# zengyan-97/X2-VLM

Hardware: AMD Instinct MI355X
Metric: image-text pairs/sec (fwd+bwd) X2VLM-base 224px bs=64/GPU (higher is better)
Workload: dtype bf16

## Files before the change

x2-vlm_amd/csrc/rowwise.hip:

```cpp
#include "x2_common.h"

__device__ __forceinline__ long remap_row(int r, int period) { return period > 0 ? (long)r + r / period + 1 : r; }

#define LN_MAXV 8
#define LN_DISPATCH(D, CALL) do { const int nv_ = ((D) + 255) / 256; \
  if (nv_ <= 1) { CALL(1); } else if (nv_ == 2) { CALL(2); } else if (nv_ == 3) { CALL(3); } else if (nv_ == 4) { CALL(4); } \
  else if (nv_ <= 6) { CALL(6); } else { CALL(8); } } while (0)
template <int NV>
__global__ __launch_bounds__(256) void layernorm_fwd_kernel(const float* __restrict__ x, const float* __restrict__ w,
                                                            const float* __restrict__ bsh, bf16_t* yb, float* yf,
                                                            float* mean, float* rstd, int rows, int D, float eps, int period,
                                                            DropSpec drop_in_, const uint32_t* __restrict__ epoch) {
  const int row = blockIdx.x * 4 + (threadIdx.x >> 6), lane = threadIdx.x & 63;
  if (row >= rows) return;
  const DropSpec drop = drop_at_epoch(drop_in_, epoch);
  const long gr = remap_row(row, period);
  const float* xr = x + gr * D;
  float4 v[NV];
  float s = 0.f;
  const int nv = D >> 2;
#pragma unroll
  for (int i = 0; i < NV; ++i) {
    const int c = lane + i * 64;
    if (c < nv) { v[i] = *reinterpret_cast<const float4*>(xr + c * 4); s += v[i].x + v[i].y + v[i].z + v[i].w; }
  }
  const float mu = wave_sum(s) / D;
  float q = 0.f;
#pragma unroll
  for (int i = 0; i < NV; ++i) {
    const int c = lane + i * 64;
    if (c < nv) { const float a = v[i].x - mu, b = v[i].y - mu, cc = v[i].z - mu, d = v[i].w - mu; q += a * a + b * b + cc * cc + d * d; }
  }
  const float rs = rsqrtf(wave_sum(q) / D + eps);
  if (lane == 0) { mean[row] = mu; rstd[row] = rs; }
#pragma unroll
  for (int i = 0; i < NV; ++i) {
    const int c = lane + i * 64;
    if (c < nv) {
      const float4 ww = *reinterpret_cast<const float4*>(w + c * 4), bb = *reinterpret_cast<const float4*>(bsh + c * 4);
      float4 o{(v[i].x - mu) * rs * ww.x + bb.x, (v[i].y - mu) * rs * ww.y + bb.y, (v[i].z - mu) * rs * ww.z + bb.z, (v[i].w - mu) * rs * ww.w + bb.w};
      if (drop.thr16) {
        float dm[4];
        drop_mul4(drop, (uint32_t)gr * (uint32_t)D + (uint32_t)(c * 4), dm);
        o.x *= dm[0]; o.y *= dm[1]; o.z *= dm[2]; o.w *= dm[3];
      }
      if (yf) *reinterpret_cast<float4*>(yf + gr * D + c * 4) = o;
      if (yb) *reinterpret_cast<u32x2*>(yb + gr * D + c * 4) = u32x2{pack_bf16(o.x, o.y), pack_bf16(o.z, o.w)};
    }
  }
}

template <int NV, int RPW>
__global__ __launch_bounds__(256) void layernorm_fwd_rows_kernel(const float* __restrict__ x, const float* __restrict__ w,
                                                                 const float* __restrict__ bsh, bf16_t* yb, float* yf,
                                                                 float* mean, float* rstd, int rows, int D, float eps, int period,
                                                                 DropSpec drop_in_, const uint32_t* __restrict__ epoch) {
  const int row0 = (blockIdx.x * 4 + (threadIdx.x >> 6)) * RPW, lane = threadIdx.x & 63;
  if (row0 >= rows) return;
  const DropSpec drop = drop_at_epoch(drop_in_, epoch);
  const int nv = D >> 2;
  float4 v[RPW][NV];
  long gr[RPW];
#pragma unroll
  for (int r = 0; r < RPW; ++r) {
    const int row = min(row0 + r, rows - 1);
    gr[r] = remap_row(row, period);
#pragma unroll
    for (int i = 0; i < NV; ++i) {
      const int c = lane + i * 64;
      v[r][i] = c < nv ? *reinterpret_cast<const float4*>(x + gr[r] * D + c * 4) : float4{0.f, 0.f, 0.f, 0.f};
    }
  }
  float4 ww[NV], bb[NV];
#pragma unroll
  for (int i = 0; i < NV; ++i) {
    const int c = lane + i * 64;
    ww[i] = c < nv ? *reinterpret_cast<const float4*>(w + c * 4) : float4{0.f, 0.f, 0.f, 0.f};
    bb[i] = c < nv ? *reinterpret_cast<const float4*>(bsh + c * 4) : float4{0.f, 0.f, 0.f, 0.f};
  }
#pragma unroll
  for (int r = 0; r < RPW; ++r) {
    float s = 0.f;
#pragma unroll
    for (int i = 0; i < NV; ++i) if (lane + i * 64 < nv) s += v[r][i].x + v[r][i].y + v[r][i].z + v[r][i].w;
    const float mu = wave_sum(s) / D;
    float q = 0.f;
#pragma unroll
    for (int i = 0; i < NV; ++i)
      if (lane + i * 64 < nv) { const float a = v[r][i].x - mu, b = v[r][i].y - mu, cc = v[r][i].z - mu, d = v[r][i].w - mu; q += a * a + b * b + cc * cc + d * d; }
    const float rs = rsqrtf(wave_sum(q) / D + eps);
    if (row0 + r >= rows) continue;
    if (lane == 0) { mean[row0 + r] = mu; rstd[row0 + r] = rs; }
#pragma unroll
    for (int i = 0; i < NV; ++i) {
      const int c = lane + i * 64;
      if (c < nv) {
        float4 o{(v[r][i].x - mu) * rs * ww[i].x + bb[i].x, (v[r][i].y - mu) * rs * ww[i].y + bb[i].y,
                 (v[r][i].z - mu) * rs * ww[i].z + bb[i].z, (v[r][i].w - mu) * rs * ww[i].w + bb[i].w};
        if (drop.thr16) {
          float dm[4];
          drop_mul4(drop, (uint32_t)gr[r] * (uint32_t)D + (uint32_t)(c * 4), dm);
          o.x *= dm[0]; o.y *= dm[1]; o.z *= dm[2]; o.w *= dm[3];
        }
        if (yf) *reinterpret_cast<float4*>(yf + gr[r] * D + c * 4) = o;
        if (yb) *reinterpret_cast<u32x2*>(yb + gr[r] * D + c * 4) = u32x2{pack_bf16(o.x, o.y), pack_bf16(o.z, o.w)};
      }
    }
  }
}

extern "C" int x2_tune_get(int key);
extern "C" int x2_layernorm_fwd(const float* x, const float* w, const float* b, void* y_bf16, float* y_f32, float* mean,
                                float* rstd, int rows, int D, float eps, int period, unsigned drop_thr16, unsigned drop_seed,
                                float drop_scale, const unsigned* drop_epoch, void* stream) {
  X2_REQUIRE(rows > 0 && D > 0 && D % 4 == 0 && D <= 256 * LN_MAXV, "x2_layernorm_fwd: rows=%d D=%d (D%%4==0, D<=2048)", rows, D);
#define X2_LNF(NV) hipLaunchKernelGGL(layernorm_fwd_kernel<NV>, dim3((rows + 3) / 4), dim3(256), 0, (hipStream_t)stream, x, w, b, \
                     (bf16_t*)y_bf16, y_f32, mean, rstd, rows, D, eps, period, DropSpec{drop_thr16, drop_seed, drop_scale}, drop_epoch)
#define X2_LNF_R(NV, RPW) hipLaunchKernelGGL((layernorm_fwd_rows_kernel<NV, RPW>), dim3((rows + 4 * RPW - 1) / (4 * RPW)), dim3(256), 0, (hipStream_t)stream, \
                     x, w, b, (bf16_t*)y_bf16, y_f32, mean, rstd, rows, D, eps, period, DropSpec{drop_thr16, drop_seed, drop_scale}, drop_epoch)
  const int knob = x2_tune_get(13), nvv = (D + 255) / 256;
  int rpw = knob == 1 || knob == 2 || knob == 4 ? knob : (rows >= 8 * 4 * 256 ? 2 : 1);
  if (nvv > 4) rpw = 1;
  if (rpw == 4 && nvv <= 3) { if (nvv <= 1) X2_LNF_R(1, 4); else if (nvv == 2) X2_LNF_R(2, 4); else X2_LNF_R(3, 4); }
  else if (rpw >= 2) { if (nvv <= 1) X2_LNF_R(1, 2); else if (nvv == 2) X2_LNF_R(2, 2); else if (nvv == 3) X2_LNF_R(3, 2); else X2_LNF_R(4, 2); }
  else LN_DISPATCH(D, X2_LNF);
  return x2_check_launch("x2_layernorm_fwd");
}

__global__ __launch_bounds__(256) void reduce_partials_kernel(const float* __restrict__ part, int nblk, int nk, int width,
                                                              float* o0, float* o1, float* o2, float* o3 = nullptr) {
  const int c = blockIdx.x * 64 + (threadIdx.x & 63), k = blockIdx.y, sl = threadIdx.x >> 6;
  __shared__ float red[3][64];
  float s = 0.f;
  if (c < width) {
#pragma unroll 4
    for (int b = sl; b < nblk; b += 4) s += part[((long)b * nk + k) * width + c];
  }
  if (sl > 0) red[sl - 1][threadIdx.x & 63] = s;
  __syncthreads();
  if (sl == 0 && c < width) {
    float* o = k == 0 ? o0 : (k == 1 ? o1 : (k == 2 ? o2 : o3));
    if (o) o[c] += s + red[0][threadIdx.x] + red[1][threadIdx.x] + red[2][threadIdx.x];
  }
}
static void launch_reduce(const float* part, int nblk, int nk, int width, float* o0, float* o1, float* o2, hipStream_t st, float* o3 = nullptr) {
  hipLaunchKernelGGL(reduce_partials_kernel, dim3((width + 63) / 64, nk), dim3(256), 0, st, part, nblk, nk, width, o0, o1, o2, o3);
}
extern "C" int x2_reduce_partials(const float* part, int nblk, int nk, int width, float* o0, float* o1, float* o2, void* stream) {
  X2_REQUIRE(part && nblk > 0 && nk >= 1 && nk <= 3 && width > 0, "x2_reduce_partials: nblk=%d nk=%d width=%d", nblk, nk, width);
  launch_reduce(part, nblk, nk, width, o0, o1, o2, (hipStream_t)stream);
  return x2_check_launch("x2_reduce_partials");
}

#define RPM_MAX 16
struct ReduceDesc { const float* part; float* o[4]; int nblk, nk, width, blk0; };
struct ReduceGroup { ReduceDesc d[RPM_MAX]; int count; };
#define RPM_COLS 16
__global__ __launch_bounds__(256) void reduce_partials_multi_kernel(ReduceGroup g) {
  int e = 0;
#pragma unroll
  for (int i = 1; i < RPM_MAX; ++i) if (i < g.count && (int)blockIdx.x >= g.d[i].blk0) e = i;
  const ReduceDesc d = g.d[e];
  const int local = blockIdx.x - d.blk0, ctiles = (d.width + RPM_COLS - 1) / RPM_COLS;
  const int k = local / ctiles, cg = threadIdx.x & 3, sl = threadIdx.x >> 2;
  const int c = (local % ctiles) * RPM_COLS + cg * 4;
  __shared__ float4 red[63][4];
  float4 s = float4{0.f, 0.f, 0.f, 0.f};
  float* o = d.o[k];
  const bool vec = (d.width & 3) == 0;
  if (o && c < d.width) {
    const float* base = d.part + (size_t)k * d.width + c;
    const size_t rs = (size_t)d.nk * d.width;
    if (vec) {
      int b = sl;
      for (; b + 192 < d.nblk; b += 256) {
        const float4 v0 = *reinterpret_cast<const float4*>(base + (size_t)b * rs), v1 = *reinterpret_cast<const float4*>(base + (size_t)(b + 64) * rs),
                     v2 = *reinterpret_cast<const float4*>(base + (size_t)(b + 128) * rs), v3 = *reinterpret_cast<const float4*>(base + (size_t)(b + 192) * rs);
        s.x += (v0.x + v1.x) + (v2.x + v3.x); s.y += (v0.y + v1.y) + (v2.y + v3.y);
        s.z += (v0.z + v1.z) + (v2.z + v3.z); s.w += (v0.w + v1.w) + (v2.w + v3.w);
      }
      for (; b < d.nblk; b += 64) {
        const float4 v = *reinterpret_cast<const float4*>(base + (size_t)b * rs);
        s.x += v.x; s.y += v.y; s.z += v.z; s.w += v.w;
      }
    } else {
      for (int b = sl; b < d.nblk; b += 64) {
        const float* r = base + (size_t)b * rs;
        s.x += r[0]; if (c + 1 < d.width) s.y += r[1]; if (c + 2 < d.width) s.z += r[2]; if (c + 3 < d.width) s.w += r[3];
      }
    }
  }
  if (sl > 0) red[sl - 1][cg] = s;
  __syncthreads();
  if (sl == 0 && o && c < d.width) {
#pragma unroll 9
    for (int i = 0; i < 63; ++i) { const float4 v = red[i][cg]; s.x += v.x; s.y += v.y; s.z += v.z; s.w += v.w; }
    o[c] += s.x;
    if (c + 1 < d.width) o[c + 1] += s.y;
    if (c + 2 < d.width) o[c + 2] += s.z;
    if (c + 3 < d.width) o[c + 3] += s.w;
  }
}
extern "C" int x2_reduce_partials_multi(const int64_t* desc, int count, void* stream) {
  X2_REQUIRE(desc && count >= 1, "x2_reduce_partials_multi: count=%d", count);
  for (int i0 = 0; i0 < count; i0 += RPM_MAX) {
    ReduceGroup g; g.count = count - i0 < RPM_MAX ? count - i0 : RPM_MAX;
    int blocks = 0;
    for (int i = 0; i < g.count; ++i) {
      const int64_t* q = desc + (size_t)(i0 + i) * 8;
      ReduceDesc& d = g.d[i];
      d.part = (const float*)q[0]; d.nblk = (int)q[1]; d.nk = (int)q[2]; d.width = (int)q[3];
      d.o[0] = (float*)q[4]; d.o[1] = (float*)q[5]; d.o[2] = (float*)q[6]; d.o[3] = (float*)q[7];
      X2_REQUIRE(d.part && d.nblk > 0 && d.nk >= 1 && d.nk <= 4 && d.width > 0, "x2_reduce_partials_multi[%d]: nblk=%d nk=%d width=%d",
                 i0 + i, d.nblk, d.nk, d.width);
      d.blk0 = blocks;
      blocks += ((d.width + RPM_COLS - 1) / RPM_COLS) * d.nk;
    }
    hipLaunchKernelGGL(reduce_partials_multi_kernel, dim3(blocks), dim3(256), 0, (hipStream_t)stream, g);
  }
  return x2_check_launch("x2_reduce_partials_multi");
}

#define LNB_ROWS 16
template <int NV, int MODE>
__global__ __launch_bounds__(256, NV <= 3 ? 4 : 1) void layernorm_bwd_kernel(const void* __restrict__ dy_, const float* __restrict__ x,
                                                            const float* __restrict__ mean, const float* __restrict__ rstd,
                                                            const float* __restrict__ w, const float* dres, float* dx, bf16_t* dxb,
                                                            float* ws, int rows, int D, int period,
                                                            DropSpec din_, DropSpec dout_, const uint32_t* __restrict__ epoch,
                                                            const float* __restrict__ post_rs) {
  constexpr int NSET = 3;
  constexpr bool DYB = MODE != 0;
  extern __shared__ __attribute__((aligned(16))) float red[];
  const DropSpec din = drop_at_epoch(din_, epoch), dout = drop_at_epoch(dout_, epoch);
  const int lane = threadIdx.x & 63, wv = threadIdx.x >> 6;
  const int nv = D >> 2;
  float4 ww[NV], aw[NV], ab[NV], ac[NV];
#pragma unroll
  for (int i = 0; i < NV; ++i) {
    const int c = lane + i * 64;
    ww[i] = c < nv ? *reinterpret_cast<const float4*>(w + c * 4) : float4{0.f, 0.f, 0.f, 0.f};
    aw[i] = float4{0.f, 0.f, 0.f, 0.f}; ab[i] = float4{0.f, 0.f, 0.f, 0.f}; ac[i] = float4{0.f, 0.f, 0.f, 0.f};
  }
  const int r0 = blockIdx.x * LNB_ROWS, r1 = min(rows, r0 + LNB_ROWS);
  for (int row = r0 + wv; row < r1; row += 4) {
    const long gr = remap_row(row, period);
    const float mu = mean[row], rs = rstd[row];
    float4 g[NV], xh[NV];
    float s1 = 0.f, s2 = 0.f;
#pragma unroll
    for (int i = 0; i < NV; ++i) {
      const int c = lane + i * 64;
      if (c < nv) {
        float4 d;
        if constexpr (DYB) {
          const u32x2 raw = *reinterpret_cast<const u32x2*>(reinterpret_cast<const bf16_t*>(dy_) + gr * D + c * 4);
          d = float4{bf_lo(raw.x), bf_hi(raw.x), bf_lo(raw.y), bf_hi(raw.y)};
        } else {
          d = *reinterpret_cast<const float4*>(reinterpret_cast<const float*>(dy_) + gr * D + c * 4);
        }
        const float4 xv = *reinterpret_cast<const float4*>(x + gr * D + c * 4);
        if (din.thr16) {
          float dm[4];
          drop_mul4(din, (uint32_t)gr * (uint32_t)D + (uint32_t)(c * 4), dm);
          d.x *= dm[0]; d.y *= dm[1]; d.z *= dm[2]; d.w *= dm[3];
        }
        xh[i] = float4{(xv.x - mu) * rs, (xv.y - mu) * rs, (xv.z - mu) * rs, (xv.w - mu) * rs};
        g[i] = float4{d.x * ww[i].x, d.y * ww[i].y, d.z * ww[i].z, d.w * ww[i].w};
        s1 += g[i].x + g[i].y + g[i].z + g[i].w;
        s2 += g[i].x * xh[i].x + g[i].y * xh[i].y + g[i].z * xh[i].z + g[i].w * xh[i].w;
        aw[i].x += d.x * xh[i].x; aw[i].y += d.y * xh[i].y; aw[i].z += d.z * xh[i].z; aw[i].w += d.w * xh[i].w;
        ab[i].x += d.x; ab[i].y += d.y; ab[i].z += d.z; ab[i].w += d.w;
      }
    }
    const float m1 = wave_sum(s1) / D, m2 = wave_sum(s2) / D;
#pragma unroll
    for (int i = 0; i < NV; ++i) {
      const int c = lane + i * 64;
      if (c < nv) {
        float4 o{rs * (g[i].x - m1 - xh[i].x * m2), rs * (g[i].y - m1 - xh[i].y * m2), rs * (g[i].z - m1 - xh[i].z * m2), rs * (g[i].w - m1 - xh[i].w * m2)};
        float4 om = o;
        if (dout.thr16) {
          float dm[4];
          drop_mul4(dout, (uint32_t)gr * (uint32_t)D + (uint32_t)(c * 4), dm);
          om.x *= dm[0]; om.y *= dm[1]; om.z *= dm[2]; om.w *= dm[3];
        }
        if (dres) { const float4 rr = *reinterpret_cast<const float4*>(dres + gr * D + c * 4); o.x += rr.x; o.y += rr.y; o.z += rr.z; o.w += rr.w; }
        if (dx) *reinterpret_cast<float4*>(dx + gr * D + c * 4) = o;
        if constexpr (MODE == 2) { om = o; if (post_rs) { const float f = post_rs[gr]; om.x *= f; om.y *= f; om.z *= f; om.w *= f; } }
        ac[i].x += om.x; ac[i].y += om.y; ac[i].z += om.z; ac[i].w += om.w;
        if (dxb) *reinterpret_cast<u32x2*>(dxb + gr * D + c * 4) = u32x2{pack_bf16(om.x, om.y), pack_bf16(om.z, om.w)};
      }
    }
  }
  if (wv > 0) {
#pragma unroll
    for (int i = 0; i < NV; ++i) {
      const int c = lane + i * 64;
      if (c < nv) {
        *reinterpret_cast<float4*>(red + ((0 * 3 + wv - 1) * D) + c * 4) = aw[i];
        *reinterpret_cast<float4*>(red + ((1 * 3 + wv - 1) * D) + c * 4) = ab[i];
        *reinterpret_cast<float4*>(red + ((2 * 3 + wv - 1) * D) + c * 4) = ac[i];
      }
    }
  }
  __syncthreads();
  if (wv == 0) {
#pragma unroll
    for (int i = 0; i < NV; ++i) {
      const int c = lane + i * 64;
      if (c < nv) {
#pragma unroll
        for (int k = 0; k < 3; ++k) {
          const float4 a = *reinterpret_cast<const float4*>(red + ((0 * 3 + k) * D) + c * 4), b = *reinterpret_cast<const float4*>(red + ((1 * 3 + k) * D) + c * 4),
                       cc = *reinterpret_cast<const float4*>(red + ((2 * 3 + k) * D) + c * 4);
          aw[i].x += a.x; aw[i].y += a.y; aw[i].z += a.z; aw[i].w += a.w;
          ab[i].x += b.x; ab[i].y += b.y; ab[i].z += b.z; ab[i].w += b.w;
          ac[i].x += cc.x; ac[i].y += cc.y; ac[i].z += cc.z; ac[i].w += cc.w;
        }
        float* wp = ws + (long)blockIdx.x * NSET * D + c * 4;
        *reinterpret_cast<float4*>(wp) = aw[i];
        *reinterpret_cast<float4*>(wp + D) = ab[i];
        *reinterpret_cast<float4*>(wp + 2 * D) = ac[i];
      }
    }
  }
}

extern "C" int x2_layernorm_bwd(const void* dy, int dy_is_bf16, const float* x, const float* mean, const float* rstd, const float* w,
                                const float* dres, float* dx, void* dx_bf16, float* dw, float* db, float* dcol, int rows, int D,
                                int period, unsigned in_thr16, unsigned in_seed, float in_scale, unsigned out_thr16,
                                unsigned out_seed, float out_scale, const unsigned* drop_epoch, float* ws, int defer, int post,
                                const float* post_rowscale, void* stream) {
  X2_REQUIRE(rows > 0 && D > 0 && D % 4 == 0 && D <= 256 * LN_MAXV, "x2_layernorm_bwd: rows=%d D=%d", rows, D);
  X2_REQUIRE(dw && db && ws, "x2_layernorm_bwd: dw/db and the workspace ws[ceil(rows/%d)*3*D] are required", LNB_ROWS);
  X2_REQUIRE(post || !(dcol && dres), "x2_layernorm_bwd: dcol sums the LN-input gradient, which excludes dres (post = 0)");
  X2_REQUIRE(!(out_thr16 && dres), "x2_layernorm_bwd: an output mask applies to the bf16 copy, which excludes dres");
  X2_REQUIRE(!post || (dy_is_bf16 && dx_bf16 && dcol && !out_thr16 && period == 0),
             "x2_layernorm_bwd: post = 1 (by-products of the final output) takes a bf16 dy, dx_bf16 and dcol, no output mask, period 0");
#define X2_LNB_T(NV, B) hipLaunchKernelGGL((layernorm_bwd_kernel<NV, B>), dim3((rows + LNB_ROWS - 1) / LNB_ROWS), dim3(256), 9 * D * sizeof(float), \
                     (hipStream_t)stream, dy, x, mean, rstd, w, dres, dx, (bf16_t*)dx_bf16, ws, rows, D, period,                \
                     DropSpec{in_thr16, in_seed, in_scale}, DropSpec{out_thr16, out_seed, out_scale}, drop_epoch, post_rowscale)
#define X2_LNB(NV) do { if (post) X2_LNB_T(NV, 2); else if (dy_is_bf16) X2_LNB_T(NV, 1); else X2_LNB_T(NV, 0); } while (0)
  LN_DISPATCH(D, X2_LNB);
  if (!defer) launch_reduce(ws, (rows + LNB_ROWS - 1) / LNB_ROWS, 3, D, dw, db, dcol, (hipStream_t)stream);
  return x2_check_launch("x2_layernorm_bwd");
}

#define CS_ROWS 64
__global__ __launch_bounds__(256) void colsum_bf16_kernel(const bf16_t* __restrict__ y, float* ws, int M, int N, int ld) {
  __shared__ float red[3][512];
  const int tx = threadIdx.x & 63, ty = threadIdx.x >> 6;
  const int c0 = blockIdx.y * 512 + tx * 8;
  const int r0 = blockIdx.x * CS_ROWS, r1 = min(M, r0 + CS_ROWS);
  float acc[8] = {0.f, 0.f, 0.f, 0.f, 0.f, 0.f, 0.f, 0.f};
  if (c0 < N) {
#pragma unroll 4
    for (int r = r0 + ty; r < r1; r += 4) {
      const u32x4 v = *reinterpret_cast<const u32x4*>(y + (long)r * ld + c0);
#pragma unroll
      for (int e = 0; e < 4; ++e) { acc[2 * e] += bf_lo(v[e]); acc[2 * e + 1] += bf_hi(v[e]); }
    }
  }
  if (ty > 0) {
#pragma unroll
    for (int e = 0; e < 8; ++e) red[ty - 1][tx * 8 + e] = acc[e];
  }
  __syncthreads();
  if (ty == 0 && c0 < N) {
#pragma unroll
    for (int e = 0; e < 8; ++e) {
      const float v = acc[e] + red[0][tx * 8 + e] + red[1][tx * 8 + e] + red[2][tx * 8 + e];
      if (c0 + e < N) ws[(long)blockIdx.x * N + c0 + e] = v;
    }
  }
}
extern "C" int x2_colsum_bf16(const void* y, float* out, int M, int N, int ld, float* ws, int defer, void* stream) {
  X2_REQUIRE(M > 0 && N > 0 && N % 8 == 0 && ld % 8 == 0, "x2_colsum_bf16: M=%d N=%d ld=%d (N, ld multiples of 8)", M, N, ld);
  X2_REQUIRE(ws, "x2_colsum_bf16: workspace ws[ceil(M/%d)*N] required", CS_ROWS);
  hipLaunchKernelGGL(colsum_bf16_kernel, dim3((M + CS_ROWS - 1) / CS_ROWS, (N + 511) / 512), dim3(256), 0, (hipStream_t)stream,
                     (const bf16_t*)y, ws, M, N, ld);
  if (!defer) launch_reduce(ws, (M + CS_ROWS - 1) / CS_ROWS, 1, N, out, nullptr, nullptr, (hipStream_t)stream);
  return x2_check_launch("x2_colsum_bf16");
}

#define LS_ROWS 32
__global__ __launch_bounds__(256) void rowscale_cast_colsum_kernel(const float* __restrict__ dx, const float* __restrict__ rowscale,
                                                                   bf16_t* dxb, float* ws, int M, int D) {
  __shared__ float red[3][256];
  const int tx = threadIdx.x & 63, ty = threadIdx.x >> 6;
  const int c0 = blockIdx.y * 256 + tx * 4;
  const int r0 = blockIdx.x * LS_ROWS, r1 = min(M, r0 + LS_ROWS);
  float ab[4] = {0.f, 0.f, 0.f, 0.f};
  if (c0 < D) {
#pragma unroll 4
    for (int r = r0 + ty; r < r1; r += 4) {
      float4 d = *reinterpret_cast<const float4*>(dx + (long)r * D + c0);
      if (rowscale) { const float rs_ = rowscale[r]; d.x *= rs_; d.y *= rs_; d.z *= rs_; d.w *= rs_; }
      *reinterpret_cast<u32x2*>(dxb + (long)r * D + c0) = u32x2{pack_bf16(d.x, d.y), pack_bf16(d.z, d.w)};
      ab[0] += d.x; ab[1] += d.y; ab[2] += d.z; ab[3] += d.w;
    }
  }
  if (ty > 0) {
#pragma unroll
    for (int e = 0; e < 4; ++e) red[ty - 1][tx * 4 + e] = ab[e];
  }
  __syncthreads();
  if (ty == 0 && c0 < D) {
#pragma unroll
    for (int e = 0; e < 4; ++e) ws[(long)blockIdx.x * D + c0 + e] = ab[e] + red[0][tx * 4 + e] + red[1][tx * 4 + e] + red[2][tx * 4 + e];
  }
}
extern "C" int x2_rowscale_cast_colsum(const float* dx, const float* rowscale, void* dx_bf16, float* colsum, int M, int D, float* ws,
                                       int defer, void* stream) {
  X2_REQUIRE(dx && dx_bf16 && colsum && M > 0 && D > 0 && D % 4 == 0 && ws,
             "x2_rowscale_cast_colsum: M=%d D=%d (workspace ws[ceil(M/%d)*D] required)", M, D, LS_ROWS);
  hipLaunchKernelGGL(rowscale_cast_colsum_kernel, dim3((M + LS_ROWS - 1) / LS_ROWS, (D + 255) / 256), dim3(256), 0, (hipStream_t)stream, dx,
                     rowscale, (bf16_t*)dx_bf16, ws, M, D);
  if (!defer) launch_reduce(ws, (M + LS_ROWS - 1) / LS_ROWS, 1, D, colsum, nullptr, nullptr, (hipStream_t)stream);
  return x2_check_launch("x2_rowscale_cast_colsum");
}

#define LSF_MAX 8
struct LsfDesc { float* G; const float* W; const float* bias; const float* gamma; const float* cs; float* dgamma; float* dbias; int N, K, blk0; };
struct LsfGroup { LsfDesc d[LSF_MAX]; int count; };
__global__ __launch_bounds__(256) void layerscale_finish_kernel(LsfGroup g) {
  int e = 0;
#pragma unroll
  for (int i = 1; i < LSF_MAX; ++i) if (i < g.count && (int)blockIdx.x >= g.d[i].blk0) e = i;
  const LsfDesc d = g.d[e];
  const int n = (blockIdx.x - d.blk0) * 4 + (threadIdx.x >> 6), lane = threadIdx.x & 63;
  if (n >= d.N) return;
  float* gr = d.G + (size_t)n * d.K;
  const float* wr = d.W + (size_t)n * d.K;
  const float gm = d.gamma[n];
  float dot = 0.f;
  for (int k = lane * 4; k < d.K; k += 256) {
    float4 gv = *reinterpret_cast<const float4*>(gr + k);
    const float4 wv = *reinterpret_cast<const float4*>(wr + k);
    dot += gv.x * wv.x + gv.y * wv.y + gv.z * wv.z + gv.w * wv.w;
    gv.x *= gm; gv.y *= gm; gv.z *= gm; gv.w *= gm;
    *reinterpret_cast<float4*>(gr + k) = gv;
  }
  dot = wave_sum(dot);
  if (lane == 0) {
    const float c = d.cs[n];
    d.dgamma[n] += dot + (d.bias ? d.bias[n] * c : 0.f);
    if (d.dbias) d.dbias[n] += gm * c;
  }
}
extern "C" int x2_layerscale_finish(const int64_t* desc, int count, void* stream) {
  X2_REQUIRE(desc && count >= 1, "x2_layerscale_finish: count=%d", count);
  for (int i0 = 0; i0 < count; i0 += LSF_MAX) {
    LsfGroup g; g.count = count - i0 < LSF_MAX ? count - i0 : LSF_MAX;
    int blocks = 0;
    for (int i = 0; i < g.count; ++i) {
      const int64_t* q = desc + (size_t)(i0 + i) * 9;
      LsfDesc& d = g.d[i];
      d.G = (float*)q[0]; d.W = (const float*)q[1]; d.bias = (const float*)q[2]; d.gamma = (const float*)q[3]; d.cs = (const float*)q[4];
      d.dgamma = (float*)q[5]; d.dbias = (float*)q[6]; d.N = (int)q[7]; d.K = (int)q[8];
      X2_REQUIRE(d.G && d.W && d.gamma && d.cs && d.dgamma && d.N > 0 && d.K > 0 && d.K % 4 == 0, "x2_layerscale_finish[%d]: N=%d K=%d", i0 + i,
                 d.N, d.K);
      d.blk0 = blocks;
      blocks += (d.N + 3) / 4;
    }
    hipLaunchKernelGGL(layerscale_finish_kernel, dim3(blocks), dim3(256), 0, (hipStream_t)stream, g);
  }
  return x2_check_launch("x2_layerscale_finish");
}

__global__ __launch_bounds__(256) void cast_bf16_kernel(const float* __restrict__ s, bf16_t* __restrict__ d, long n4) {
  long i = blockIdx.x * 256L + threadIdx.x;
  const long st = (long)gridDim.x * 256;
  for (; i < n4; i += st) {
    const float4 v = *reinterpret_cast<const float4*>(s + i * 4);
    *reinterpret_cast<u32x2*>(d + i * 4) = u32x2{pack_bf16(v.x, v.y), pack_bf16(v.z, v.w)};
  }
}
extern "C" int x2_cast_bf16(const float* src, void* dst, long n, void* stream) {
  X2_REQUIRE(n > 0 && n % 4 == 0, "x2_cast_bf16: n=%ld must be a positive multiple of 4", n);
  const long n4 = n / 4;
  const int blocks = (int)((n4 + 255) / 256 < 4096 ? (n4 + 255) / 256 : 4096);
  hipLaunchKernelGGL(cast_bf16_kernel, dim3(blocks), dim3(256), 0, (hipStream_t)stream, src, (bf16_t*)dst, n4);
  return x2_check_launch("x2_cast_bf16");
}

__global__ __launch_bounds__(256) void cast_transpose_kernel(const float* __restrict__ s, bf16_t* d, bf16_t* dT, int R, int C, int ldt) {
  __shared__ float tile[64][65];
  const int r0 = blockIdx.y * 64, c0 = blockIdx.x * 64;
  const int tx = threadIdx.x & 15, ty = threadIdx.x >> 4;
  const bool vec = ((C | ldt | R) & 3) == 0;
#pragma unroll
  for (int i = 0; i < 4; ++i) {
    const int r = r0 + ty + 16 * i, c = c0 + tx * 4;
    float4 v{0.f, 0.f, 0.f, 0.f};
    if (r < R) {
      if (vec && c + 3 < C) {
        v = *reinterpret_cast<const float4*>(s + (long)r * C + c);
// ... 329 lines not shown
```

x2-vlm_amd/kernels.py:

```python
import ctypes as C

import torch

from . import _lib
from ._lib import AttnArgs, call, ptr, raw_stream

BF16, F32 = torch.bfloat16, torch.float32


GEMM_TIMER = None


class _timed:

    def __init__(self, flops, name="gemm_nt"):
        self.flops = flops
        self.name = name

    def __enter__(self):
        if GEMM_TIMER is not None:
            self.a = torch.cuda.Event(enable_timing=True)
            self.b = torch.cuda.Event(enable_timing=True)
            self.a.record()

# ... 134 lines not shown
    return out


def gemm_nt_splitk(A, B, out=None, slices=0):
    assert A.dtype == BF16 and B.dtype == BF16 and A.shape[1] == B.shape[1]
    M, K = A.shape
    N = B.shape[0]
    if out is None:
        out = torch.empty(M, N, device=A.device, dtype=F32)
    assert out.shape == (M, N) and out.dtype == F32
    ws = workspace(A.device, min(32, max(1, K // 64)) * M * N)
    with _timed(2.0 * M * N * K):
        call("x2_gemm_nt_splitk", ptr(A), ptr(B), ptr(out), M, N, K, _rows(A), _rows(B), _rows(out), slices, ptr(ws), ws.numel())
    return out


def gemm_tn_grouped(problems, accumulate=False, split=0):
    rows = []
    for pr in problems:
        dY, X, dW = pr[:3]
        assert dY.dtype == BF16 and X.dtype == BF16 and dW.dtype == F32 and dY.shape[0] == X.shape[0]
        N, K = dW.shape
        n_ld, k_ld = (pr[3], pr[4]) if len(pr) == 5 else (dY.shape[1], X.shape[1])
        assert dY.shape[1] >= N or n_ld >= N
        rows.append([dY.data_ptr(), X.data_ptr(), dW.data_ptr(), dY.shape[0], N, K, _rows(dY), _rows(X), _rows(dW),
                     n_ld, k_ld])
    dev = problems[0][0].device
    for i in range(0, len(rows), 8):
        chunk = rows[i:i + 8]
        arr = (C.c_int64 * (11 * len(chunk)))(*[v for r in chunk for v in r])
        tiles256 = sum(((r[4] + 255) // 256) * ((r[5] + 255) // 256) for r in chunk)
        want = (split if split else 4) * tiles256 * 65536
        ws = workspace(dev, want) if split != 1 else None
        with _timed(sum(2.0 * r[3] * r[4] * r[5] for r in chunk), "gemm_tn"):
            call("x2_gemm_tn_grouped", arr, len(chunk), 1 if accumulate else 0, split, ptr(ws), 0 if ws is None else ws.numel())



def _attn_args(q, k, v, B, Bkv, H, Lq, Lk, scale, bias=None, biasT=None, mask=None, kv_idx=None, seq_off=None,
               seq_ids=None, drop=NO_DROP, head_dim=64, bias_log2=False):
    a = AttnArgs()
    a.Q, a.q_bs, a.q_rs = q
    a.K, a.k_bs, a.k_rs = k
    a.V, a.v_bs, a.v_rs = v
    a.B, a.Bkv, a.H, a.Lq, a.Lk, a.scale = B, Bkv, H, Lq, Lk, scale
    a.head_dim = head_dim
    a.dbg = 16 if bias_log2 else 0
    a.drop_thr16, a.drop_seed, a.drop_scale = drop[:3]
    a.drop_epoch = ptr(drop[3])
    if bias is not None:
        assert bias.dtype == F32 and bias.dim() == 3 and bias.is_contiguous()
        a.bias, a.bias_ld = bias.data_ptr(), bias.shape[2]
    if biasT is not None:
        assert biasT.dtype == F32 and biasT.dim() == 3 and biasT.is_contiguous()
        a.biasT, a.biasT_ld = biasT.data_ptr(), biasT.shape[2]
    if mask is not None:
        assert mask.dtype == F32 and mask.dim() == 2 and mask.is_contiguous() and mask.shape[0] == B
        a.mask, a.mask_ld = mask.data_ptr(), mask.shape[1]
    if kv_idx is not None:
        assert kv_idx.dtype == torch.int32 and kv_idx.numel() == B
        a.kv_idx = kv_idx.data_ptr()
    if seq_off is not None:
        assert seq_off.dtype == torch.int32 and seq_ids.dtype == torch.int32
        a.seq_off, a.seq_ids = seq_off.data_ptr(), seq_ids.data_ptr()
    return a


def view3(t, B, L, col0=0):
    assert t.dtype == BF16 and t.dim() == 2 and t.stride(1) == 1 and t.shape[0] == B * L
    return (t.data_ptr() + 2 * col0, L * t.stride(0), t.stride(0))


def attn_fwd(q, k, v, B, Bkv, H, Lq, Lk, scale, out, lse, **kw):
    a = _attn_args(q, k, v, B, Bkv, H, Lq, Lk, scale, **kw)
    a.Out, a.o_bs, a.o_rs = out
    assert lse.dtype == F32 and lse.numel() == B * H * Lq
    a.LSE = lse.data_ptr()
    call("x2_attn_fwd", C.byref(a))


def attn_bwd_form(Lq, Lk, shared_kv=False, dropout=False, workspace=False):
    a = AttnArgs()
    a.B = a.Bkv = a.H = 1
    a.Lq, a.Lk, a.head_dim, a.scale = Lq, Lk, 64, 0.125
    for f in ("q_bs", "q_rs", "k_bs", "k_rs", "v_bs", "v_rs", "o_bs", "o_rs", "dq_bs", "dq_rs", "dk_bs", "dk_rs", "dv_bs", "dv_rs", "do_bs", "do_rs"):
        setattr(a, f, 64)
    if shared_kv:
        a.kv_idx = a.seq_off = a.seq_ids = 8
    a.drop_thr16 = 1 if dropout else 0
    if workspace:
        a.ws, a.ws_floats = 8, ((Lq + 127) // 128) * 8192
    return _lib.lib().x2_attn_bwd_one_pass(C.byref(a))


def attn_bwd(q, k, v, o, do, B, Bkv, H, Lq, Lk, scale, lse, delta, dq, dk, dv, dS=None, phase=0, ask_form=False, colsum_ws=None, **kw):
    a = _attn_args(q, k, v, B, Bkv, H, Lq, Lk, scale, **kw)
    a.phase = phase
    a.O, a.o_bs, a.o_rs = o
    a.dO, a.do_bs, a.do_rs = do
    a.dQ, a.dq_bs, a.dq_rs = dq
    a.dK, a.dk_bs, a.dk_rs = dk
    a.dV, a.dv_bs, a.dv_rs = dv
    a.LSE, a.Delta = lse.data_ptr(), delta.data_ptr()
    if dS is not None:
        assert dS.dtype == BF16 and dS.is_contiguous() and dS.shape[:3] == (B, H, Lq)
        a.dS, a.ds_ld = dS.data_ptr(), dS.shape[3]
    if phase == 0 and Lq > 208 and Lk > 208 and a.kv_idx is None and not a.drop_thr16:
        ws = workspace(lse.device, B * H * ((Lq + 127) // 128) * 8192)
        a.ws, a.ws_floats = ws.data_ptr(), ws.numel()
    if ask_form:
        return _lib.lib().x2_attn_bwd_one_pass(C.byref(a))
    if colsum_ws is not None:
        assert colsum_ws.dtype == F32 and colsum_ws.is_contiguous() and colsum_ws.shape == (B, 2, H * 64)
        form = _lib.lib().x2_attn_bwd_one_pass(C.byref(a))
        if form in (1, 3):
            a.colsum_ws = colsum_ws.data_ptr()
        call("x2_attn_bwd", C.byref(a))
        return form
    call("x2_attn_bwd", C.byref(a))



def layernorm_fwd(x, w, b, eps, *, rows=None, period=0, want_bf16=True, want_f32=False, y_bf16=None, y_f32=None,
                  drop=NO_DROP):
    assert x.dtype == F32 and x.is_contiguous()
    D = x.shape[-1]
    x2 = x.view(-1, D)
    R = x2.shape[0] if rows is None else rows
    if want_bf16 and y_bf16 is None:
        y_bf16 = torch.empty_like(x2, dtype=BF16)
    if want_f32 and y_f32 is None:
        y_f32 = torch.empty_like(x2)
    mean = torch.empty(R, device=x.device, dtype=F32)
    rstd = torch.empty(R, device=x.device, dtype=F32)
    call("x2_layernorm_fwd", ptr(x2), ptr(w), ptr(b), ptr(y_bf16), ptr(y_f32), ptr(mean), ptr(rstd), R, D, eps, period,
         drop[0], drop[1], drop[2], ptr(drop[3]))
    return y_bf16, y_f32, mean, rstd


def layernorm_bwd(dy, x, mean, rstd, w, dw, db, *, dres=None, dcol=None, period=0, want_f32=True, want_bf16=False, dx=None,
                  drop_in=NO_DROP, drop_out=NO_DROP, post=None):
    assert dy.dtype in (F32, BF16) and x.dtype == F32 and dy.is_contiguous() and x.is_contiguous()
    D = x.shape[-1]
    R = mean.numel()
    if want_f32 and dx is None:
        dx = torch.empty_like(x) if period == 0 else torch.zeros_like(x)
    prs = None
    if post is not None:
        assert dcol is None and dy.dtype == BF16 and period == 0
        prs, dcol = post
        assert prs is None or (prs.dtype == F32 and prs.numel() == R and prs.is_contiguous())
        want_bf16 = True
    dxb = torch.empty(x.shape, device=x.device, dtype=BF16) if want_bf16 else None
    nblk = (R + 15) // 16
    ws, defer = _ws_and_defer(x.device, nblk * 3 * D)
    call("x2_layernorm_bwd", ptr(dy), 1 if dy.dtype == BF16 else 0, ptr(x), ptr(mean), ptr(rstd), ptr(w), ptr(dres), ptr(dx), ptr(dxb), ptr(dw), ptr(db),
         ptr(dcol), R, D, period, drop_in[0], drop_in[1], drop_in[2], drop_out[0], drop_out[1], drop_out[2],
         ptr(drop_in[3] if drop_in[3] is not None else drop_out[3]), ptr(ws), defer, 0 if post is None else 1, ptr(prs))
    if defer:
        DEFERRED.append((ws, nblk, 3, D, (dw, db, dcol)))
    return dx, dxb


def colsum_bf16(y, out):
    nblk = (y.shape[0] + 63) // 64
    ws, defer = _ws_and_defer(y.device, nblk * y.shape[1])
    call("x2_colsum_bf16", ptr(y), ptr(out), y.shape[0], y.shape[1], _rows(y), ptr(ws), defer)
    if defer:
        DEFERRED.append((ws, nblk, 1, y.shape[1], (out,)))


def rowscale_cast_colsum(dx, colsum, rowscale=None):
    assert dx.dtype == F32 and dx.is_contiguous() and dx.dim() == 2
    dxb = torch.empty_like(dx, dtype=BF16)
    nblk = (dx.shape[0] + 31) // 32
    ws, defer = _ws_and_defer(dx.device, nblk * dx.shape[1])
    call("x2_rowscale_cast_colsum", ptr(dx), ptr(rowscale), ptr(dxb), ptr(colsum), dx.shape[0], dx.shape[1], ptr(ws), defer)
    if defer:
        DEFERRED.append((ws, nblk, 1, dx.shape[1], (colsum,)))
    return dxb


def layerscale_finish(items):
    flat = []
    for G, W, bias, gamma, cs, dgamma, dbias in items:
        N, Kd = G.shape
        assert G.dtype == F32 and W.dtype == F32 and G.is_contiguous() and W.is_contiguous() and W.numel() == G.numel() and Kd % 4 == 0
        flat += [G.data_ptr(), W.data_ptr(), 0 if bias is None else bias.data_ptr(), gamma.data_ptr(), cs.data_ptr(), dgamma.data_ptr(),
                 0 if dbias is None else dbias.data_ptr(), N, Kd]
    call("x2_layerscale_finish", (C.c_int64 * len(flat))(*flat), len(items))


def cast_bf16(src, out=None):
    assert src.dtype == F32 and src.is_contiguous() and src.numel() % 4 == 0
    if out is None:
        out = torch.empty_like(src, dtype=BF16)
    call("x2_cast_bf16", ptr(src), ptr(out), src.numel())
    return out


def cast_transpose_bf16(src, want_plain=True, ldt=None):
    assert src.dtype == F32 and src.dim() == 2 and src.is_contiguous()
    R, Cc = src.shape
    ldt = R if ldt is None else ldt
    plain = torch.empty(R, Cc, device=src.device, dtype=BF16) if want_plain else None
    tr = (torch.zeros if ldt > R else torch.empty)(Cc, ldt, device=src.device, dtype=BF16)
    call("x2_cast_transpose_bf16", ptr(src), ptr(plain), ptr(tr), R, Cc, ldt)
    return plain, tr


def patchify(image, ps):
    assert image.dtype == F32 and image.is_contiguous() and image.dim() == 4 and image.shape[1] == 3
    B, _, R, _ = image.shape
    g = R // ps
    cols = torch.empty(B * g * g, 3 * ps * ps, device=image.device, dtype=BF16)
    call("x2_patchify", ptr(image), ptr(cols), B, R, ps)
    return cols


def assemble_tokens(patch, cls, B, P):
    D = patch.shape[1]
    x = torch.empty(B, P + 1, D, device=patch.device, dtype=F32)
    call("x2_assemble_tokens", ptr(patch), ptr(cls), ptr(x), B, P, D)
    return x


def assemble_tokens_bwd(dx, dcls):
    B, T, D = dx.shape
    dpatch = torch.empty(B * (T - 1), D, device=dx.device, dtype=BF16)
    call("x2_assemble_tokens_bwd", ptr(dx), ptr(dpatch), ptr(dcls), B, T - 1, D)
    return dpatch


def pool_tokens(x, w=None, bwd=False):
    B, T, D = x.shape
    assert x.dtype == F32 and x.is_contiguous() and (w is None or (w.dtype == F32 and w.shape == (B, T - 1) and w.is_contiguous()))
    call("x2_pool_tokens", ptr(x), ptr(w), B, T - 1, D, 1 if bwd else 0)
    return x


LOG2E = 1.4426950408889634


def relpos_bias(table, index, want_T=True, log2=False):
    N = index.shape[0]
    H = table.shape[1]
    ld = round_up(N, 64)
    bias = torch.empty(H, N, ld, device=table.device, dtype=F32)
    biasT = torch.empty(H, N, ld, device=table.device, dtype=F32) if want_T else None
    call("x2_relpos_bias", ptr(table), ptr(index), ptr(_relpos_index_t(index)) if want_T else None, ptr(bias), ptr(biasT), N, H, ld, ld,
         LOG2E if log2 else 1.0)
    return bias, biasT


_RELPOS_CSR = {}
_RELPOS_T = {}


def _relpos_index_t(index):
    key = (index.data_ptr(), index._version)
    ent = _RELPOS_T.get(key)
    if ent is None:
        ent = _RELPOS_T[key] = (index.t().contiguous(), index)
    return ent[0]



def _relpos_csr(index, ld, T):
    key = (index.data_ptr(), index._version, ld, T)
    ent = _RELPOS_CSR.get(key)
    if ent is None:
        N = index.shape[0]
        flat = index.reshape(-1)
        order = torch.argsort(flat, stable=True)
        off = torch.zeros(T + 1, device=index.device, dtype=torch.int32)
        off[1:] = torch.cumsum(torch.bincount(flat, minlength=T), 0)
        pos = ((order // N) * ld + order % N).to(torch.int32).contiguous()
        ent = _RELPOS_CSR[key] = (off, pos, index)
    return ent[0], ent[1]


def relpos_bias_bwd(dS, index, dtable):
    B, H, N, ld = dS.shape
    T = dtable.shape[0]
    assert dS.dtype == BF16 and dS.is_contiguous() and dtable.dtype == F32 and dtable.is_contiguous() and dtable.shape[1] == H
    off, pos = _relpos_csr(index, ld, T)
    slices = 1
    ws = workspace(dS.device, slices * H * N * ld)
    call("x2_relpos_bias_bwd", ptr(dS), ptr(off), ptr(pos), ptr(dtable), B, N, H, ld, T, ptr(ws), slices)



def embed_fwd(ids, word, pos, type_emb):
    R, L = ids.numel(), ids.shape[-1]
    D = word.shape[1]
    out = torch.empty(R, D, device=word.device, dtype=F32)
    call("x2_embed_fwd", ptr(ids), ptr(word), ptr(pos), ptr(type_emb), ptr(out), R, L, D)
    return out


def embed_bwd(ids, g, dword, dpos, dtype):
    R, L = ids.numel(), ids.shape[-1]
    D = g.shape[-1]
    scratch = workspace(g.device, min(L, R) * D)
    call("x2_embed_bwd", ptr(ids), ptr(g), ptr(dword), ptr(dpos), ptr(dtype), R, L, D, ptr(scratch))


# ... 204 lines not shown
```

Before: 2945.

## Cap LayerNorm backward blocks, prefetch rows, and unify partial-sum reduction kernel

LayerNorm backward now launches at most 512 blocks, each covering several rows, so fewer per-block partials are written and reduced. Inside the kernel the next row's dy, x, mean and rstd are fetched while the current row is computed. The old single reduce kernel is removed in favour of the multi kernel, which now handles 32 columns per block and unrolls the load loop eight ways. The risks are higher register pressure from the prefetch buffers (the launch-bounds occupancy hint drops to 2) and less parallelism in the LN backward grid.

```diff
diff --git a/x2-vlm_amd/csrc/rowwise.hip b/x2-vlm_amd/csrc/rowwise.hip
--- a/x2-vlm_amd/csrc/rowwise.hip
+++ b/x2-vlm_amd/csrc/rowwise.hip
@@ -127,44 +127,21 @@
   return x2_check_launch("x2_layernorm_fwd");
 }
 
-__global__ __launch_bounds__(256) void reduce_partials_kernel(const float* __restrict__ part, int nblk, int nk, int width,
-                                                              float* o0, float* o1, float* o2, float* o3 = nullptr) {
-  const int c = blockIdx.x * 64 + (threadIdx.x & 63), k = blockIdx.y, sl = threadIdx.x >> 6;
-  __shared__ float red[3][64];
-  float s = 0.f;
-  if (c < width) {
-#pragma unroll 4
-    for (int b = sl; b < nblk; b += 4) s += part[((long)b * nk + k) * width + c];
-  }
-  if (sl > 0) red[sl - 1][threadIdx.x & 63] = s;
-  __syncthreads();
-  if (sl == 0 && c < width) {
-    float* o = k == 0 ? o0 : (k == 1 ? o1 : (k == 2 ? o2 : o3));
-    if (o) o[c] += s + red[0][threadIdx.x] + red[1][threadIdx.x] + red[2][threadIdx.x];
-  }
-}
-static void launch_reduce(const float* part, int nblk, int nk, int width, float* o0, float* o1, float* o2, hipStream_t st, float* o3 = nullptr) {
-  hipLaunchKernelGGL(reduce_partials_kernel, dim3((width + 63) / 64, nk), dim3(256), 0, st, part, nblk, nk, width, o0, o1, o2, o3);
-}
-extern "C" int x2_reduce_partials(const float* part, int nblk, int nk, int width, float* o0, float* o1, float* o2, void* stream) {
-  X2_REQUIRE(part && nblk > 0 && nk >= 1 && nk <= 3 && width > 0, "x2_reduce_partials: nblk=%d nk=%d width=%d", nblk, nk, width);
-  launch_reduce(part, nblk, nk, width, o0, o1, o2, (hipStream_t)stream);
-  return x2_check_launch("x2_reduce_partials");
-}
-
 #define RPM_MAX 16
 struct ReduceDesc { const float* part; float* o[4]; int nblk, nk, width, blk0; };
 struct ReduceGroup { ReduceDesc d[RPM_MAX]; int count; };
-#define RPM_COLS 16
+#define RPM_COLS 32
+#define RPM_CG (RPM_COLS / 4)
+#define RPM_SL (256 / RPM_CG)
 __global__ __launch_bounds__(256) void reduce_partials_multi_kernel(ReduceGroup g) {
   int e = 0;
 #pragma unroll
   for (int i = 1; i < RPM_MAX; ++i) if (i < g.count && (int)blockIdx.x >= g.d[i].blk0) e = i;
   const ReduceDesc d = g.d[e];
   const int local = blockIdx.x - d.blk0, ctiles = (d.width + RPM_COLS - 1) / RPM_COLS;
-  const int k = local / ctiles, cg = threadIdx.x & 3, sl = threadIdx.x >> 2;
+  const int k = local / ctiles, cg = threadIdx.x % RPM_CG, sl = threadIdx.x / RPM_CG;
   const int c = (local % ctiles) * RPM_COLS + cg * 4;
-  __shared__ float4 red[63][4];
+  __shared__ float4 red[RPM_SL - 1][RPM_CG];
   float4 s = float4{0.f, 0.f, 0.f, 0.f};
   float* o = d.o[k];
   const bool vec = (d.width & 3) == 0;
@@ -172,19 +149,18 @@
     const float* base = d.part + (size_t)k * d.width + c;
     const size_t rs = (size_t)d.nk * d.width;
     if (vec) {
-      int b = sl;
-      for (; b + 192 < d.nblk; b += 256) {
-        const float4 v0 = *reinterpret_cast<const float4*>(base + (size_t)b * rs), v1 = *reinterpret_cast<const float4*>(base + (size_t)(b + 64) * rs),
-                     v2 = *reinterpret_cast<const float4*>(base + (size_t)(b + 128) * rs), v3 = *reinterpret_cast<const float4*>(base + (size_t)(b + 192) * rs);
-        s.x += (v0.x + v1.x) + (v2.x + v3.x); s.y += (v0.y + v1.y) + (v2.y + v3.y);
-        s.z += (v0.z + v1.z) + (v2.z + v3.z); s.w += (v0.w + v1.w) + (v2.w + v3.w);
-      }
-      for (; b < d.nblk; b += 64) {
-        const float4 v = *reinterpret_cast<const float4*>(base + (size_t)b * rs);
-        s.x += v.x; s.y += v.y; s.z += v.z; s.w += v.w;
+      for (int b = sl; b < d.nblk; b += 8 * RPM_SL) {
+        float4 v[8];
+#pragma unroll
+        for (int j = 0; j < 8; ++j)
+          v[j] = b + j * RPM_SL < d.nblk ? *reinterpret_cast<const float4*>(base + (size_t)(b + j * RPM_SL) * rs) : float4{0.f, 0.f, 0.f, 0.f};
+        s.x += ((v[0].x + v[1].x) + (v[2].x + v[3].x)) + ((v[4].x + v[5].x) + (v[6].x + v[7].x));
+        s.y += ((v[0].y + v[1].y) + (v[2].y + v[3].y)) + ((v[4].y + v[5].y) + (v[6].y + v[7].y));
+        s.z += ((v[0].z + v[1].z) + (v[2].z + v[3].z)) + ((v[4].z + v[5].z) + (v[6].z + v[7].z));
+        s.w += ((v[0].w + v[1].w) + (v[2].w + v[3].w)) + ((v[4].w + v[5].w) + (v[6].w + v[7].w));
       }
     } else {
-      for (int b = sl; b < d.nblk; b += 64) {
+      for (int b = sl; b < d.nblk; b += RPM_SL) {
         const float* r = base + (size_t)b * rs;
         s.x += r[0]; if (c + 1 < d.width) s.y += r[1]; if (c + 2 < d.width) s.z += r[2]; if (c + 3 < d.width) s.w += r[3];
       }
@@ -193,13 +169,25 @@
   if (sl > 0) red[sl - 1][cg] = s;
   __syncthreads();
   if (sl == 0 && o && c < d.width) {
-#pragma unroll 9
-    for (int i = 0; i < 63; ++i) { const float4 v = red[i][cg]; s.x += v.x; s.y += v.y; s.z += v.z; s.w += v.w; }
+#pragma unroll
+    for (int i = 0; i < RPM_SL - 1; ++i) { const float4 v = red[i][cg]; s.x += v.x; s.y += v.y; s.z += v.z; s.w += v.w; }
     o[c] += s.x;
     if (c + 1 < d.width) o[c + 1] += s.y;
     if (c + 2 < d.width) o[c + 2] += s.z;
     if (c + 3 < d.width) o[c + 3] += s.w;
   }
+}
+static int reduce_blocks(const ReduceDesc& d) { return ((d.width + RPM_COLS - 1) / RPM_COLS) * d.nk; }
+static void launch_reduce(const float* part, int nblk, int nk, int width, float* o0, float* o1, float* o2, hipStream_t st) {
+  ReduceGroup g;
+  g.count = 1;
+  g.d[0] = ReduceDesc{part, {o0, o1, o2, nullptr}, nblk, nk, width, 0};
+  hipLaunchKernelGGL(reduce_partials_multi_kernel, dim3(reduce_blocks(g.d[0])), dim3(256), 0, st, g);
+}
+extern "C" int x2_reduce_partials(const float* part, int nblk, int nk, int width, float* o0, float* o1, float* o2, void* stream) {
+  X2_REQUIRE(part && nblk > 0 && nk >= 1 && nk <= 3 && width > 0, "x2_reduce_partials: nblk=%d nk=%d width=%d", nblk, nk, width);
+  launch_reduce(part, nblk, nk, width, o0, o1, o2, (hipStream_t)stream);
+  return x2_check_launch("x2_reduce_partials");
 }
 extern "C" int x2_reduce_partials_multi(const int64_t* desc, int count, void* stream) {
   X2_REQUIRE(desc && count >= 1, "x2_reduce_partials_multi: count=%d", count);
@@ -214,7 +202,7 @@
       X2_REQUIRE(d.part && d.nblk > 0 && d.nk >= 1 && d.nk <= 4 && d.width > 0, "x2_reduce_partials_multi[%d]: nblk=%d nk=%d width=%d",
                  i0 + i, d.nblk, d.nk, d.width);
       d.blk0 = blocks;
-      blocks += ((d.width + RPM_COLS - 1) / RPM_COLS) * d.nk;
+      blocks += reduce_blocks(d);
     }
     hipLaunchKernelGGL(reduce_partials_multi_kernel, dim3(blocks), dim3(256), 0, (hipStream_t)stream, g);
   }
@@ -222,11 +210,13 @@
 }
 
 #define LNB_ROWS 16
+#define LNB_MAXBLK 512
+static inline int lnb_blocks(int rows) { const int b = (rows + LNB_ROWS - 1) / LNB_ROWS; return b < LNB_MAXBLK ? b : LNB_MAXBLK; }
 template <int NV, int MODE>
-__global__ __launch_bounds__(256, NV <= 3 ? 4 : 1) void layernorm_bwd_kernel(const void* __restrict__ dy_, const float* __restrict__ x,
+__global__ __launch_bounds__(256, NV <= 4 ? 2 : 1) void layernorm_bwd_kernel(const void* __restrict__ dy_, const float* __restrict__ x,
                                                             const float* __restrict__ mean, const float* __restrict__ rstd,
                                                             const float* __restrict__ w, const float* dres, float* dx, bf16_t* dxb,
-                                                            float* ws, int rows, int D, int period,
+                                                            float* ws, int rows, int D, int period, int per,
                                                             DropSpec din_, DropSpec dout_, const uint32_t* __restrict__ epoch,
                                                             const float* __restrict__ post_rs) {
   constexpr int NSET = 3;
@@ -242,24 +232,51 @@
     ww[i] = c < nv ? *reinterpret_cast<const float4*>(w + c * 4) : float4{0.f, 0.f, 0.f, 0.f};
     aw[i] = float4{0.f, 0.f, 0.f, 0.f}; ab[i] = float4{0.f, 0.f, 0.f, 0.f}; ac[i] = float4{0.f, 0.f, 0.f, 0.f};
   }
-  const int r0 = blockIdx.x * LNB_ROWS, r1 = min(rows, r0 + LNB_ROWS);
-  for (int row = r0 + wv; row < r1; row += 4) {
+  const int r0 = blockIdx.x * per, r1 = min(rows, r0 + per);
+  u32x2 pb[NV];
+  float4 pf[NV], px[NV];
+  float pmu = 0.f, prs = 0.f;
+  auto fetch = [&](int row) {
     const long gr = remap_row(row, period);
-    const float mu = mean[row], rs = rstd[row];
-    float4 g[NV], xh[NV];
-    float s1 = 0.f, s2 = 0.f;
 #pragma unroll
     for (int i = 0; i < NV; ++i) {
       const int c = lane + i * 64;
       if (c < nv) {
-        float4 d;
-        if constexpr (DYB) {
-          const u32x2 raw = *reinterpret_cast<const u32x2*>(reinterpret_cast<const bf16_t*>(dy_) + gr * D + c * 4);
-          d = float4{bf_lo(raw.x), bf_hi(raw.x), bf_lo(raw.y), bf_hi(raw.y)};
-        } else {
-          d = *reinterpret_cast<const float4*>(reinterpret_cast<const float*>(dy_) + gr * D + c * 4);
-        }
-        const float4 xv = *reinterpret_cast<const float4*>(x + gr * D + c * 4);
+        if constexpr (DYB) pb[i] = *reinterpret_cast<const u32x2*>(reinterpret_cast<const bf16_t*>(dy_) + gr * D + c * 4);
+        else pf[i] = *reinterpret_cast<const float4*>(reinterpret_cast<const float*>(dy_) + gr * D + c * 4);
+        px[i] = *reinterpret_cast<const float4*>(x + gr * D + c * 4);
+      }
+    }
+    pmu = mean[row]; prs = rstd[row];
+  };
+  if (r0 + wv < r1) fetch(r0 + wv);
+  for (int row = r0 + wv; row < r1; row += 4) {
+    const long gr = remap_row(row, period);
+    const float mu = pmu, rs = prs;
+    float4 d4[NV], xv4[NV], rr[NV];
+#pragma unroll
+    for (int i = 0; i < NV; ++i) {
+      if constexpr (DYB) d4[i] = float4{bf_lo(pb[i].x), bf_hi(pb[i].x), bf_lo(pb[i].y), bf_hi(pb[i].y)};
+      else d4[i] = pf[i];
+      xv4[i] = px[i];
+    }
+    if (dres) {
+#pragma unroll
+      for (int i = 0; i < NV; ++i) {
+        const int c = lane + i * 64;
+        if (c < nv) rr[i] = *reinterpret_cast<const float4*>(dres + gr * D + c * 4);
+      }
+    }
+    const float prow = MODE == 2 && post_rs ? post_rs[gr] : 1.f;
+    if (row + 4 < r1) fetch(row + 4);
+    float4 g[NV], xh[NV];
+    float s1 = 0.f, s2 = 0.f;
+#pragma unroll
+    for (int i = 0; i < NV; ++i) {
+      const int c = lane + i * 64;
+      if (c < nv) {
+        float4 d = d4[i];
+        const float4 xv = xv4[i];
         if (din.thr16) {
           float dm[4];
           drop_mul4(din, (uint32_t)gr * (uint32_t)D + (uint32_t)(c * 4), dm);
@@ -285,9 +302,9 @@
           drop_mul4(dout, (uint32_t)gr * (uint32_t)D + (uint32_t)(c * 4), dm);
           om.x *= dm[0]; om.y *= dm[1]; om.z *= dm[2]; om.w *= dm[3];
         }
-        if (dres) { const float4 rr = *reinterpret_cast<const float4*>(dres + gr * D + c * 4); o.x += rr.x; o.y += rr.y; o.z += rr.z; o.w += rr.w; }
+        if (dres) { o.x += rr[i].x; o.y += rr[i].y; o.z += rr[i].z; o.w += rr[i].w; }
         if (dx) *reinterpret_cast<float4*>(dx + gr * D + c * 4) = o;
-        if constexpr (MODE == 2) { om = o; if (post_rs) { const float f = post_rs[gr]; om.x *= f; om.y *= f; om.z *= f; om.w *= f; } }
+        if constexpr (MODE == 2) { om = o; if (post_rs) { om.x *= prow; om.y *= prow; om.z *= prow; om.w *= prow; } }
         ac[i].x += om.x; ac[i].y += om.y; ac[i].z += om.z; ac[i].w += om.w;
         if (dxb) *reinterpret_cast<u32x2*>(dxb + gr * D + c * 4) = u32x2{pack_bf16(om.x, om.y), pack_bf16(om.z, om.w)};
       }
@@ -333,17 +350,18 @@
                                 unsigned out_seed, float out_scale, const unsigned* drop_epoch, float* ws, int defer, int post,
                                 const float* post_rowscale, void* stream) {
   X2_REQUIRE(rows > 0 && D > 0 && D % 4 == 0 && D <= 256 * LN_MAXV, "x2_layernorm_bwd: rows=%d D=%d", rows, D);
-  X2_REQUIRE(dw && db && ws, "x2_layernorm_bwd: dw/db and the workspace ws[ceil(rows/%d)*3*D] are required", LNB_ROWS);
+  X2_REQUIRE(dw && db && ws, "x2_layernorm_bwd: dw/db and the workspace ws[min(ceil(rows/%d), %d)*3*D] are required", LNB_ROWS, LNB_MAXBLK);
   X2_REQUIRE(post || !(dcol && dres), "x2_layernorm_bwd: dcol sums the LN-input gradient, which excludes dres (post = 0)");
   X2_REQUIRE(!(out_thr16 && dres), "x2_layernorm_bwd: an output mask applies to the bf16 copy, which excludes dres");
   X2_REQUIRE(!post || (dy_is_bf16 && dx_bf16 && dcol && !out_thr16 && period == 0),
              "x2_layernorm_bwd: post = 1 (by-products of the final output) takes a bf16 dy, dx_bf16 and dcol, no output mask, period 0");
-#define X2_LNB_T(NV, B) hipLaunchKernelGGL((layernorm_bwd_kernel<NV, B>), dim3((rows + LNB_ROWS - 1) / LNB_ROWS), dim3(256), 9 * D * sizeof(float), \
-                     (hipStream_t)stream, dy, x, mean, rstd, w, dres, dx, (bf16_t*)dx_bf16, ws, rows, D, period,                \
+  const int nblk = lnb_blocks(rows), per = (rows + nblk - 1) / nblk;
+#define X2_LNB_T(NV, B) hipLaunchKernelGGL((layernorm_bwd_kernel<NV, B>), dim3(nblk), dim3(256), 9 * D * sizeof(float), \
+                     (hipStream_t)stream, dy, x, mean, rstd, w, dres, dx, (bf16_t*)dx_bf16, ws, rows, D, period, per,           \
                      DropSpec{in_thr16, in_seed, in_scale}, DropSpec{out_thr16, out_seed, out_scale}, drop_epoch, post_rowscale)
 #define X2_LNB(NV) do { if (post) X2_LNB_T(NV, 2); else if (dy_is_bf16) X2_LNB_T(NV, 1); else X2_LNB_T(NV, 0); } while (0)
   LN_DISPATCH(D, X2_LNB);
-  if (!defer) launch_reduce(ws, (rows + LNB_ROWS - 1) / LNB_ROWS, 3, D, dw, db, dcol, (hipStream_t)stream);
+  if (!defer) launch_reduce(ws, nblk, 3, D, dw, db, dcol, (hipStream_t)stream);
   return x2_check_launch("x2_layernorm_bwd");
 }
 
diff --git a/x2-vlm_amd/kernels.py b/x2-vlm_amd/kernels.py
--- a/x2-vlm_amd/kernels.py
+++ b/x2-vlm_amd/kernels.py
@@ -310,7 +310,7 @@
         assert prs is None or (prs.dtype == F32 and prs.numel() == R and prs.is_contiguous())
         want_bf16 = True
     dxb = torch.empty(x.shape, device=x.device, dtype=BF16) if want_bf16 else None
-    nblk = (R + 15) // 16
+    nblk = min((R + 15) // 16, 512)
     ws, defer = _ws_and_defer(x.device, nblk * 3 * D)
     call("x2_layernorm_bwd", ptr(dy), 1 if dy.dtype == BF16 else 0, ptr(x), ptr(mean), ptr(rstd), ptr(w), ptr(dres), ptr(dx), ptr(dxb), ptr(dw), ptr(db),
          ptr(dcol), R, D, period, drop_in[0], drop_in[1], drop_in[2], drop_out[0], drop_out[1], drop_out[2],
```

After: 2977, median of 6. +1.1%, better.
